# xmengli/H-DenseUNet

Measured on AMD Instinct MI355X. Metric: CT slices/sec fwd+bwd (2D 512^2), higher is better.
Workload: dtype bf16

## Files before the change

### h-denseunet_amd/csrc/conv_igemm.hip

```cpp
#include "conv_common.h"
#include "../../include/hdu.h"

template <typename T, int BM, int BN> struct BnbGeom {
  static constexpr int CH = Chunk<T>::CH;
  static constexpr int NCC = BN / CH;
  static constexpr int NCCP = NCC <= 4 ? 4 : (NCC <= 8 ? 8 : (NCC <= 16 ? 16 : 32));
  static constexpr int RSTEP = 256 / NCCP;
  static constexpr int IT = (BM + RSTEP - 1) / RSTEP;
  static constexpr bool EARLY = IT <= 8;
  static_assert(NCC <= 32, "tile shape");
};

template <bool SPLIT, typename T, int BM, int BN, int WAVES_M, int WAVES_N>
__device__ __forceinline__ void conv_igemm_body(const ConvK& p, char* smem) {
  constexpr int CH = Chunk<T>::CH;
  constexpr int BK = 8 * CH;
  constexpr int A_IT = BM / 32;
  constexpr int B_IT = (BN + 31) / 32;
  constexpr int WM = BM / WAVES_M;
  constexpr int WN = BN / WAVES_N;
  constexpr int TM = WM / 16;
  constexpr int TN = WN / 16;
  constexpr int STAGE = (BM + BN) * 128;
  static_assert(WAVES_M * WAVES_N == 4, "4 waves");
// ... 1571 lines not shown
          if constexpr (PRO) {
            const int cb = kt * BK + chunk * CH;
#pragma unroll
            for (int i = 0; i < TM; ++i) af[i] = pro_apply<T>(af[i], pro_ta + cb, pro_tb + cb, pro_lo);
          }
#pragma unroll
          for (int i = 0; i < TM; ++i)
#pragma unroll
            for (int j = 0; j < TN; ++j) acc[i][j] = Mma<T>::kgroup(bf[j], af[i], acc[i][j]);
        }
        if (!issue_first) issue(slot == 0 ? NS - 1 : slot - 1);
        slot = slot == NS - 1 ? 0 : slot + 1;
      }
      const int n0 = nt * BN;
      float* sdst = p.stats_partial ? p.stats_partial + (long long)((unsigned)mt % (unsigned)p.stats_slots) * 2 * p.Cout : nullptr;
#pragma unroll
      for (int j = 0; j < TN; ++j) {
        const int n = n0 + j * 16 + (lane >> 4) * 4;
        const bool n_ok = n < p.Cout;
        const int nc = n_ok ? n : 0;
        const f32x4 bias_v = has_bias ? *(const f32x4*)(p.bias + nc) : f32x4{0.f, 0.f, 0.f, 0.f};
        const f32x4 epa_v = has_epi ? *(const f32x4*)(p.epi_a + nc) : f32x4{1.f, 1.f, 1.f, 1.f};
        const f32x4 epb_v = has_epi ? *(const f32x4*)(p.epi_b + nc) : f32x4{0.f, 0.f, 0.f, 0.f};
        const f32x4 sh_v = sdst ? *(const f32x4*)(p.stats_shift + nc) : f32x4{0.f, 0.f, 0.f, 0.f};
        float s1[4] = {0.f, 0.f, 0.f, 0.f}, s2[4] = {0.f, 0.f, 0.f, 0.f};
#pragma unroll
        for (int i = 0; i < TM; ++i) {
          const long long m = (long long)mt * BM + wave * WM + i * 16 + (lane & 15);
          const bool ok = n_ok && m < p.M;
          T* dst = yp + (ok ? m * p.ldy + n : 0);
          float v[4] = {acc[i][j][0], acc[i][j][1], acc[i][j][2], acc[i][j][3]};
          if (has_bias) {
#pragma unroll
            for (int r = 0; r < 4; ++r) v[r] += bias_v[r];
          }
          if (drop) {
#pragma unroll
            for (int r = 0; r < 4; ++r) {
              const unsigned h = hdu_hash32((unsigned long long)m * (unsigned)p.Cout + (unsigned)(n + r), dseed);
              v[r] = h < p.drop_thresh ? v[r] * p.drop_scale : 0.f;
            }
          }
          if (has_epi) {
#pragma unroll
            for (int r = 0; r < 4; ++r) {
              v[r] = epa_v[r] * v[r] + epb_v[r];
              if (p.epi_relu) v[r] = v[r] > 0.f ? v[r] : 0.f;
            }
          }
          if (p.accumulate) {
            float old[4];
            Chunk<T>::load4(dst, old);
#pragma unroll
            for (int r = 0; r < 4; ++r) v[r] += old[r];
          }
          if (ok) Chunk<T>::store4(dst, v);
          if (sdst) {
#pragma unroll
            for (int r = 0; r < 4; ++r) {
              const float d = ok ? Chunk<T>::rounded(v[r]) - sh_v[r] : 0.f;
              s1[r] += d;
              s2[r] += d * d;
            }
          }
        }
        if (sdst) {
#pragma unroll
          for (int r = 0; r < 4; ++r) { s1[r] = hdu_row16_sum(s1[r]); s2[r] = hdu_row16_sum(s2[r]); }
          const int q = lane & 15;
          float mine = 0.f;
#pragma unroll
          for (int r = 0; r < 4; ++r) {
            mine = q == r ? s1[r] : mine;
            mine = q == 4 + r ? s2[r] : mine;
          }
          if (q < 8 && n_ok) atomicAdd(sdst + (q < 4 ? 0 : p.Cout) + n + (q & 3), mine);
        }
      }
    }
  }
  HDU_WAIT_VMCNT(0);
}

template <int KS, int BN, bool BNB = false, int NSA = 3>
__global__ __launch_bounds__(256) void conv_pw_bstat_kernel(ConvK p, int rows_per_wg) {
  typedef bf16_t T;
  constexpr int CH = 8, BM = 64;
  constexpr int PD = NSA - 1;
  constexpr int A_SLAB = BM * 128, A_STAGE = KS * A_SLAB;
  constexpr int B_SLAB = BN * 128, B_BYTES = KS * B_SLAB;
  constexpr int WM = 32, WN = BN / 2, TM = WM / 16, TN = WN / 16;
  constexpr int CROWB = WN * 2 + (BN == 64 && NSA == 2 ? 0 : 16), CST = WM * CROWB;
  static_assert(NSA == 2 || NSA == 3, "ring depth");
  constexpr int A_IT = BM / 32, B_IT = BN / 32, LA = KS * A_IT;
  static_assert(BN % 64 == 0 && KS >= 1 && KS <= 4, "shape");
  static_assert(B_BYTES + NSA * A_STAGE + 4 * CST <= 160 * 1024, "LDS");
  __shared__ __attribute__((aligned(16))) char smem[B_BYTES + NSA * A_STAGE + 4 * CST];
  char* Bsm = smem;
  char* Aring = smem + B_BYTES;

  const int tid = threadIdx.x;
  const int lane = tid & 63;
#ifdef HDU_EMU
  const int wave = tid >> 6;
#else
  const int wave = __builtin_amdgcn_readfirstlane(tid >> 6);
#endif
  const int wm = wave >> 1, wn = wave & 1;
  char* stg = smem + B_BYTES + NSA * A_STAGE + wave * CST;
  const int r0 = tid >> 3;
  const int kcl = (tid & 7) ^ (r0 & 7);
  unsigned brow = blockIdx.x, bcol = blockIdx.y;
  if (!(p.debug_flags & 2048)) {
    const unsigned lin = blockIdx.y * gridDim.x + blockIdx.x;
    const unsigned tix = xcd_tile_index(lin, gridDim.x * gridDim.y);
    bcol = tix % gridDim.y;
    brow = tix / gridDim.y;
  }
  const int n0 = (int)bcol * BN;
  const long long m_begin = (long long)brow * rows_per_wg;
  long long m_end = m_begin + rows_per_wg;
  if (m_end > p.M) m_end = p.M;
  const int ntiles = (int)((m_end - m_begin + BM - 1) / BM);
  if (ntiles <= 0) return;
  const hdu_bufsrd xsrd = hdu_make_srd(p.x, p.x_bytes);
  const hdu_bufsrd wsrd = hdu_make_srd(p.w, p.w_bytes);

#pragma unroll
  for (int ks = 0; ks < KS; ++ks)
#pragma unroll
    for (int j = 0; j < B_IT; ++j) {
      const int col = n0 + r0 + j * 32;
      const unsigned off = col < p.Cout ? (unsigned)(col * p.Ktot + ks * 64 + kcl * CH) * 2u : HDU_OOB;
      hdu_bufload_lds16(wsrd, off, Bsm + ks * B_SLAB + (j * 32 + wave * 8) * 128);
    }
  auto issue_tile = [&](int t) {
    char* As = Aring + (t % NSA) * A_STAGE;
#pragma unroll
    for (int i = 0; i < A_IT; ++i) {
      const long long m = m_begin + (long long)t * BM + r0 + i * 32;
#pragma unroll
      for (int ks = 0; ks < KS; ++ks) {
        const unsigned off = m < m_end ? (unsigned)((unsigned long long)m * (unsigned long long)p.ldx + ks * 64 + kcl * CH) * 2u : HDU_OOB;
        hdu_bufload_lds16(xsrd, off, As + ks * A_SLAB + (i * 32 + wave * 8) * 128);
      }
    }
  };
  T* __restrict__ yp = (T*)p.y;
  constexpr int NCCE = WN / CH;
  constexpr int EIT = WM * NCCE / 64;
  static_assert(EIT == 4 || EIT == 2, "the counted waits below name four / two registers per operand");
  const int ecc = lane % NCCE;
  const int en = n0 + wn * WN + ecc * CH;
  const bool en_ok = en < p.Cout;
  float ba[CH], bb[CH], bmu[CH], brs[CH], bs1[CH], bs2[CH];
  const bool bsums = BNB && p.bnb_partial != nullptr;
  if constexpr (BNB) {
    const int nc = en_ok ? en : 0;
    const float* pmu = bsums ? p.bnb_mean : p.bnb_a;
    const float* prs = bsums ? p.bnb_rstd : p.bnb_a;
#pragma unroll
    for (int j = 0; j < CH; j += 4) {
      const f32x4 va = *(const f32x4*)(p.bnb_a + nc + j), vb = *(const f32x4*)(p.bnb_b + nc + j);
      const f32x4 vm = *(const f32x4*)(pmu + nc + j), vr = *(const f32x4*)(prs + nc + j);
#pragma unroll
      for (int r = 0; r < 4; ++r) { ba[j + r] = va[r]; bb[j + r] = vb[r]; bmu[j + r] = bsums ? vm[r] : 0.f; brs[j + r] = bsums ? vr[r] : 0.f; }
    }
#pragma unroll
    for (int j = 0; j < CH; ++j) { bs1[j] = 0.f; bs2[j] = 0.f; }
  }
  const T* __restrict__ bup = (const T*)p.bnb_u;

  u32x4 uS[NSA][EIT], oS[NSA][EIT];
  u32x4 pst[EIT];
  unsigned poff[EIT];
#pragma unroll
  for (int it = 0; it < EIT; ++it) { poff[it] = HDU_OOB; pst[it] = u32x4{0u, 0u, 0u, 0u}; }
  const hdu_rawsrd ysrd = hdu_make_rawsrd(p.y, (unsigned)(((p.M - 1) * p.ldy + p.Cout) * 2));
  const hdu_rawsrd usrd = hdu_make_rawsrd(BNB ? p.bnb_u : p.y, (unsigned)(((p.M - 1) * (BNB ? p.bnb_ldu : p.ldy) + p.Cout) * 2));
  const unsigned ldu2 = (unsigned)p.bnb_ldu * 2u, ldy2 = (unsigned)p.ldy * 2u;
  const int erow = lane / NCCE;
  auto issue_chunks = [&](int t, u32x4 (&uv)[EIT], u32x4 (&ov)[EIT]) {
#pragma unroll
    for (int it = 0; it < EIT; ++it) {
      const long long m = m_begin + (long long)t * BM + wm * WM + erow + it * (64 / NCCE);
      const bool ok = en_ok && m < m_end;
      const unsigned uoff = ok ? (unsigned)m * ldu2 + (unsigned)en * 2u : HDU_OOB;
      const unsigned ooff = (ok && p.accumulate) ? (unsigned)m * ldy2 + (unsigned)en * 2u : HDU_OOB;
      HDU_ASYNC_BUFLOAD16(uv[it], usrd, uoff);
      HDU_ASYNC_BUFLOAD16(ov[it], ysrd, ooff);
    }
  };
  if constexpr (BNB) issue_chunks(0, uS[0], oS[0]);
  issue_tile(0);
  if constexpr (PD == 2) {
    if constexpr (BNB) issue_chunks(1, uS[1], oS[1]);
    issue_tile(1);
  }

  auto tile = [&](int t, u32x4 (&cuv)[EIT], u32x4 (&cov)[EIT], u32x4 (&nuv)[EIT], u32x4 (&nov)[EIT]) {
    if constexpr (BNB) hdu_wait_vmcnt_n<(PD - 1) * (LA + 2 * EIT)>(); else hdu_wait_vmcnt_n<(PD - 1) * LA>();
    HDU_RAW_BARRIER();
#pragma unroll
    for (int it = 0; it < EIT; ++it) hdu_bufstore16(ysrd, poff[it], pst[it]);
    if constexpr (BNB) issue_chunks(t + PD, nuv, nov);
    issue_tile(t + PD);
    f32x4 acc[TM][TN];
#pragma unroll
    for (int i = 0; i < TM; ++i)
#pragma unroll
      for (int j = 0; j < TN; ++j) acc[i][j] = f32x4{0.f, 0.f, 0.f, 0.f};
    const char* At = Aring + (t % NSA) * A_STAGE;
#pragma unroll
    for (int ks = 0; ks < KS; ++ks) {
      const char* As = At + ks * A_SLAB;
      const char* Bs = Bsm + ks * B_SLAB;
#pragma unroll
      for (int kg = 0; kg < 2; ++kg) {
        u32x4 af[TM], bf[TN];
        const int chunk = kg * 4 + (lane >> 4);
#pragma unroll
        for (int i = 0; i < TM; ++i) af[i] = *(const u32x4*)(As + lds_chunk_off(wm * WM + i * 16 + (lane & 15), chunk));
#pragma unroll
        for (int j = 0; j < TN; ++j) bf[j] = *(const u32x4*)(Bs + lds_chunk_off(wn * WN + j * 16 + (lane & 15), chunk));
#pragma unroll
        for (int i = 0; i < TM; ++i)
#pragma unroll
          for (int j = 0; j < TN; ++j) acc[i][j] = Mma<T>::kgroup(bf[j], af[i], acc[i][j]);
      }
    }
#pragma unroll
    for (int i = 0; i < TM; ++i)
#pragma unroll
      for (int j = 0; j < TN; ++j) {
        const float v[4] = {acc[i][j][0], acc[i][j][1], acc[i][j][2], acc[i][j][3]};
        Chunk<T>::store4((T*)(stg + (i * 16 + (lane & 15)) * CROWB) + j * 16 + (lane >> 4) * 4, v);
      }
    HDU_WAVE_LDS_SYNC();
    if constexpr (BNB) {
      constexpr int NUSE = LA + PD * (LA + 2 * EIT);
      if constexpr (EIT == 4) {
        hdu_wait_vmcnt_regs4<NUSE>(cuv[0], cuv[1], cuv[2], cuv[3]);
        hdu_wait_vmcnt_regs4<NUSE>(cov[0], cov[1], cov[2], cov[3]);
      } else {
        hdu_wait_vmcnt_regs4<NUSE>(cuv[0], cuv[1], cov[0], cov[1]);
      }
    }
#pragma unroll
    for (int it = 0; it < EIT; ++it) {
      const int q = lane + it * 64;
      const int row = q / NCCE, cc = q % NCCE;
      const long long m = m_begin + (long long)t * BM + wm * WM + row;
      const int n = n0 + wn * WN + cc * CH;
      const u32x4 v = *(const u32x4*)(stg + row * CROWB + cc * 16);
      const bool ok = m < m_end && n < p.Cout;
      poff[it] = ok ? (unsigned)m * ldy2 + (unsigned)n * 2u : HDU_OOB;
      if constexpr (BNB) {
        float dz[CH], u[CH], o[CH];
        Chunk<T>::unpack(v, dz);
        Chunk<T>::unpack(cuv[it], u);
#pragma unroll
        for (int j = 0; j < CH; ++j) {
          const float sj = ba[j] * u[j] + bb[j];
          const float g = (ok && (!p.bnb_relu || sj > 0.f)) ? dz[j] : 0.f;
          bs1[j] += g;
          bs2[j] += g * ((u[j] - bmu[j]) * brs[j]);
          o[j] = ba[j] * g;
        }
        if (p.accumulate) {
          float old[CH];
          Chunk<T>::unpack(cov[it], old);
#pragma unroll
          for (int j = 0; j < CH; ++j) o[j] += old[j];
        }
        pst[it] = Chunk<T>::pack(o);
      } else {
        pst[it] = v;
      }
    }
    HDU_WAVE_LDS_SYNC();
  };
  if constexpr (NSA == 3) {
    for (int t = 0; t < ntiles; t += 3) {
      tile(t, uS[0], oS[0], uS[2], oS[2]);
      if (t + 1 < ntiles) tile(t + 1, uS[1], oS[1], uS[0], oS[0]);
      if (t + 2 < ntiles) tile(t + 2, uS[2], oS[2], uS[1], oS[1]);
    }
  } else {
    for (int t = 0; t < ntiles; t += 2) {
      tile(t, uS[0], oS[0], uS[1], oS[1]);
      if (t + 1 < ntiles) tile(t + 1, uS[1], oS[1], uS[0], oS[0]);
    }
  }
#pragma unroll
  for (int it = 0; it < EIT; ++it) hdu_bufstore16(ysrd, poff[it], pst[it]);
  hdu_wait_vmcnt_n<0>();
  if constexpr (BNB) {
    if (bsums) {
#pragma unroll
      for (int mask = NCCE; mask < 64; mask <<= 1) {
#pragma unroll
        for (int j = 0; j < CH; ++j) { bs1[j] += __shfl_xor(bs1[j], mask); bs2[j] += __shfl_xor(bs2[j], mask); }
      }
      float* dst = p.bnb_partial + (long long)(brow % (unsigned)p.bnb_slots) * 2 * p.Cout;
      if (lane < NCCE && en_ok) {
#pragma unroll
        for (int j = 0; j < CH; ++j) {
          atomicAdd(dst + en + j, bs1[j]);
          atomicAdd(dst + p.Cout + en + j, bs2[j]);
        }
      }
    }
  }
}

template <int BCO, bool PW, int NCT = 1>
__device__ __forceinline__ void wgrad_dma_body(const ConvK& p, float* __restrict__ dw, long long rows_per_split,
                                               unsigned bid, char* smem) {
  typedef bf16_t T;
  constexpr int CH = 8;
  constexpr int PX = 64;
  constexpr int BKC = 128;
  constexpr int XROWB = 256;
  constexpr int DROWB = 128;
  constexpr int TM = BCO / 16;
  constexpr int TN = 2;
  constexpr int STAGE = PX * (XROWB + NCT * DROWB);

  const int tid = threadIdx.x;
  const int lane = tid & 63;
#ifdef HDU_EMU
  const int wave = tid >> 6;
#else
  const int wave = __builtin_amdgcn_readfirstlane(tid >> 6);
#endif
  const T* __restrict__ xp = (const T*)p.x;
  const T* __restrict__ dyp = (const T*)p.y;
  const char* zero = (const char*)hdu_zero_page;
  const bool ups = (p.ud | p.uh | p.uw) != 0;

  unsigned wbx, wby, wbz;
  if (!(p.debug_flags & 256)) bid = xcd_tile_index(bid, (unsigned)(p.wg_gx * p.wg_gy * p.wg_gz));
  if (!wgrad_block(p, bid, &wbx, &wby, &wbz)) return;
  const int kcol0 = (int)wbx * BKC;
  const int co0 = (int)wby * BCO * NCT;
  const long long m_begin = (long long)wbz * rows_per_split;
  long long m_end = m_begin + rows_per_split;
  if (m_end > p.M) m_end = p.M;

  const int pxl = tid >> 4;
  const int fx = (pxl & 3) | ((pxl >> 1) & 4);
  const int xp16 = tid & 15;
  const int kcc = ((((xp16 >> 1) ^ fx) << 1) | (xp16 & 1));
  const int kk = kcol0 + kcc * CH;
  const bool kvalid = kk < p.Ktot;
  int c = 0, kd = 0, kh = 0, kw = 0;
  if (kvalid) {
    const int tap = kk / p.Cin;
    c = kk - tap * p.Cin;
    kw = tap % p.KW;
    const int t = tap / p.KW;
    kh = t % p.KH;
    kd = t / p.KH;
  }
  int sn[4], sod[4], soh[4], sow[4];
#pragma unroll
  for (int i = 0; i < 4; ++i) {
    if (PW) { sn[i] = sod[i] = soh[i] = sow[i] = 0; continue; }
    const long long m = m_begin + pxl + i * 16;
    const unsigned mu = (unsigned)m;
    const int ow = (int)(mu % (unsigned)p.Wo);
    unsigned t = mu / (unsigned)p.Wo;
    const int oh = (int)(t % (unsigned)p.Ho);
    t /= (unsigned)p.Ho;
    sod[i] = (int)(t % (unsigned)p.Do);
    sn[i] = (int)(t / (unsigned)p.Do);
    soh[i] = oh;
    sow[i] = ow;
  }
  const int dpx0 = tid >> 3;
  const int gd = ((dpx0 >> 1) & 1) | (((dpx0 >> 3) & 1) << 1);
  const int dp16 = tid & 7;
  const int dcl = ((((dp16 >> 1) ^ gd) << 1) | (dp16 & 1));
  bool dvalid[NCT];
#pragma unroll
  for (int t = 0; t < NCT; ++t) dvalid[t] = dcl * CH < BCO && co0 + t * BCO + dcl * CH < p.Cout;

  auto issue_tile = [&](int buf, long long mt) {
    char* Xt = smem + buf * STAGE;
    char* Dt = Xt + PX * XROWB;
#pragma unroll
    for (int i = 0; i < 4; ++i) {
      const long long m = mt + pxl + i * 16;
      const char* g;
      if (PW) {
        g = (kvalid && m < m_end) ? (const char*)(xp + m * p.ldx + c) : zero;
// ... 1048 lines not shown
  return items >= min_items && k.M < (1ll << 31) - 256;
}

template <typename T, int BN>
static void launch_pers(const ConvK& k, hipStream_t s) {
  const int tiles_m = (int)((k.M + 255) / 256), tiles_n = (k.Cout + BN - 1) / BN;
  const int cus = g_tuning[HDU_TUNE_PERS] > 1 ? g_tuning[HDU_TUNE_PERS] : 256;
  long long items = (long long)tiles_m * tiles_n;
  const dim3 grid((unsigned)(items < cus ? items : cus));
  if (k.pro_a != nullptr) {
    const int cap = pers_table_cap(BN, k.Cin);
    if (cap == HDU_PRO_CSMALL) {
      if constexpr (3 * (256 + BN) * 128 + 8 * HDU_PRO_CSMALL <= 160 * 1024)
        HDU_LAUNCH((conv_igemm_pers_kernel<T, BN, HDU_PRO_CSMALL>), grid, dim3(512), 0, s, k, tiles_m, tiles_n);
    } else {
      if constexpr (3 * (256 + BN) * 128 + 8 * HDU_PRO_CMAX <= 160 * 1024)
        HDU_LAUNCH((conv_igemm_pers_kernel<T, BN, HDU_PRO_CMAX>), grid, dim3(512), 0, s, k, tiles_m, tiles_n);
    }
  } else {
    HDU_LAUNCH((conv_igemm_pers_kernel<T, BN, 0>), grid, dim3(512), 0, s, k, tiles_m, tiles_n);
  }
}

template <typename T>
static void dispatch_igemm(const ConvK& k, size_t skb, hipStream_t s) {
  int bm, bn;
  choose_igemm(k, &bm, &bn);
  if (bm == 128 && igemm_pers_ok(k, bn)) {
    switch (bn) {
      case 128: launch_pers<T, 128>(k, s); return;
      case 96: launch_pers<T, 96>(k, s); return;
      case 64: launch_pers<T, 64>(k, s); return;
      case 48: launch_pers<T, 48>(k, s); return;
      default: launch_pers<T, 32>(k, s); return;
    }
  }
  if (bm == 64) dispatch_igemm_bn<T, 64>(k, bn, skb, s);
  else dispatch_igemm_bn<T, 128>(k, bn, skb, s);
}

bool hdu_halo_wide_taken(const ConvK& k, int dtype);
const char* hdu_halo_wide_name(const ConvK& k, int dtype);
bool hdu_halo_wide_launch(const ConvK& k, int dtype, hipStream_t s);
bool hdu_stem_wgrad_taken(const ConvK& k, int dtype);
bool hdu_stem_wgrad_launch(const ConvK& k, int dtype, float* dw, hipStream_t s);

static bool fprop_halo_ok(const ConvK& k, int dtype) {
  return dtype == HDU_BF16 && k.bnb_u == nullptr && !g_tuning[HDU_TUNE_NO_HALO_FPROP] && k.pro_a == nullptr && k.skip == nullptr && k.KD == 1 &&
         k.KH == 3 && k.KW == 3 && k.sd == 1 && k.sh == 1 && k.sw == 1 && k.pd == 0 && k.ph == 1 && k.pw == 1 &&
         (k.ud | k.uh | k.uw) == 0 && k.Di == 1 && k.Cin % 8 == 0 && k.We >= 32 && k.He >= 4 &&
         k.Do == 1 && k.Ho == k.He && k.Wo == k.We &&
         k.Cin >= 128 && k.Cout <= 96 &&
         (long long)k.N * ((k.He + 3) / 4) * ((k.We + 31) / 32) * k.M_layer / k.M >= (g_tuning[HDU_TUNE_HALO_MIN_TILES] > 0 ? g_tuning[HDU_TUNE_HALO_MIN_TILES] : 128);
}

static int choose_halo_bn(const ConvK& k) {
  const int cands[4] = {96, 64, 48, 32};
  int best = 64;
  long long best_cost = -1;
  for (int i = 0; i < 4; ++i) {
    const int c = cands[i];
    const long long cost = (long long)((k.Cout + c - 1) / c) * (c + 24);
    if (best_cost < 0 || cost < best_cost) { best_cost = cost; best = c; }
  }
  return best;
}

template <int BN>
static void launch_halo_fprop(const ConvK& k, hipStream_t s) {
  const unsigned tiles = (unsigned)(k.N * ((k.He + 3) / 4) * ((k.We + 31) / 32));
  HDU_LAUNCH((conv_halo_fprop_kernel<BN>), dim3(tiles, (unsigned)((k.Cout + BN - 1) / BN)), dim3(256), 0, s, k);
}

static bool pw_bstat_ok(const ConvK& k, int dtype) {
  return dtype == HDU_BF16 && !g_tuning[HDU_TUNE_NO_PW_BSTAT] && k.KD * k.KH * k.KW == 1 && k.sd == 1 && k.sh == 1 && k.sw == 1 &&
         (k.pd | k.ph | k.pw) == 0 && (k.ud | k.uh | k.uw) == 0 && k.pro_a == nullptr && k.skip == nullptr && k.bias == nullptr &&
         k.epi_a == nullptr && k.stats_partial == nullptr && (k.bnb_u != nullptr ? (!g_tuning[HDU_TUNE_NO_PW_BSTAT_BNB] && !(k.bnb_relu & 6)) : !k.accumulate) &&
         k.drop_scale == 0.f &&
         (k.Ktot == 128 || k.Ktot == 192) && k.Cout >= 256 && k.M >= 64 && k.x_bytes != 0 &&
         (k.M - 1) * k.ldy + k.Cout < (1ll << 31) && (k.bnb_u == nullptr || (k.M - 1) * k.bnb_ldu + k.Cout < (1ll << 31)) &&
         (long long)k.Cout * k.Ktot * 2 < (1ll << 31) && k.Do == k.De && k.Ho == k.He && k.Wo == k.We;
}

template <int BN, int NSA>
static void launch_pw_bstat_form(const ConvK& k, int target, hipStream_t s) {
  const unsigned ny = (unsigned)((k.Cout + BN - 1) / BN);
  long long splits = target / (long long)ny;
  if (splits < 1) splits = 1;
  const long long tiles = (k.M + 63) / 64;
  if (splits > tiles) splits = tiles;
  const long long rows = ((tiles + splits - 1) / splits) * 64;
  const unsigned gx = (unsigned)((k.M + rows - 1) / rows);
  if (k.bnb_u != nullptr) {
    if (k.Ktot == 192) HDU_LAUNCH((conv_pw_bstat_kernel<3, BN, true, NSA>), dim3(gx, ny), dim3(256), 0, s, k, (int)rows);
    else HDU_LAUNCH((conv_pw_bstat_kernel<2, BN, true, NSA>), dim3(gx, ny), dim3(256), 0, s, k, (int)rows);
    return;
  }
  if (k.Ktot == 192) HDU_LAUNCH((conv_pw_bstat_kernel<3, BN, false, NSA>), dim3(gx, ny), dim3(256), 0, s, k, (int)rows);
  else HDU_LAUNCH((conv_pw_bstat_kernel<2, BN, false, NSA>), dim3(gx, ny), dim3(256), 0, s, k, (int)rows);
}

static int pw_bstat_form(const ConvK& k) {
  const int f = g_tuning[HDU_TUNE_PW_BSTAT_FORM];
  if (f == 1 || f == 2) return f;
  return k.bnb_u != nullptr ? 2 : 1;
}

static void launch_pw_bstat(const ConvK& k, hipStream_t s) {
  const int wgs = g_tuning[HDU_TUNE_PW_BSTAT_WGS];
  if (pw_bstat_form(k) == 2) launch_pw_bstat_form<64, 2>(k, wgs > 0 ? wgs : 512, s);
  else launch_pw_bstat_form<128, 3>(k, wgs > 0 ? wgs : 256, s);
}

extern "C" int hdu_conv_fprop(const hdu_conv_desc* d, void* stream) {
  ConvK k;
  if (int e = fill_convk(d, &k, false)) return e;
  if (!d->y) return hdu_set_error(HDU_ERR_ARG, "conv_fprop: null output");
  if (k.M == 0) return 0;
  if (k.y_ds && !hdu_halo_wide_taken(k, d->dtype))
    return hdu_set_error(HDU_ERR_ARG, "conv_fprop: y_ds needs a launch that a halo-wide configuration takes");
  if (pw_bstat_ok(k, d->dtype)) {
    launch_pw_bstat(k, (hipStream_t)stream);
    return hdu_check_launch("conv_fprop(pointwise, filter-stationary)");
  }
  if (hdu_halo_wide_launch(k, d->dtype, (hipStream_t)stream)) return hdu_check_launch("conv_fprop(halo, wide)");
  if (fprop_halo_ok(k, d->dtype)) {
    switch (choose_halo_bn(k)) {
      case 96: launch_halo_fprop<96>(k, (hipStream_t)stream); break;
      case 64: launch_halo_fprop<64>(k, (hipStream_t)stream); break;
      case 48: launch_halo_fprop<48>(k, (hipStream_t)stream); break;
      default: launch_halo_fprop<32>(k, (hipStream_t)stream); break;
    }
    return hdu_check_launch("conv_fprop(halo)");
  }
  if (d->dtype == HDU_BF16) dispatch_igemm<bf16_t>(k, d->splitk_ws_bytes, (hipStream_t)stream);
  else dispatch_igemm<float>(k, d->splitk_ws_bytes, (hipStream_t)stream);
  return hdu_check_launch("conv_fprop");
}

extern "C" size_t hdu_conv_splitk_ws_bytes(const hdu_conv_desc* d) {
  ConvK k;
  if (fill_convk(d, &k, false)) return 0;
  if (k.M == 0 || pw_bstat_ok(k, d->dtype) || hdu_halo_wide_taken(k, d->dtype) || fprop_halo_ok(k, d->dtype) || (k.pro_a != nullptr && !igemm_pro_dma_ok(k)) || k.skip != nullptr) return 0;
  int bm, bn;
  choose_igemm(k, &bm, &bn);
  if (bm == 128 && igemm_pers_ok(k, bn)) return 0;
  const long long nblk = ((k.M + bm - 1) / bm) * ((k.Cout + bn - 1) / bn);
  const long long nblk_layer = ((k.M_layer + bm - 1) / bm) * ((k.Cout + bn - 1) / bn);
  const int stage = (bm + ((bn + 31) / 32) * 32) * 128;
  const int nsd = stage * 6 <= 160 * 1024 ? 6 : 4;
  if (!igemm_ring_ok(nblk_layer, k.Ktot, stage, nsd)) return 0;
  const int bk = d->dtype == HDU_BF16 ? 64 : 32;
  size_t need;
  choose_splitk(nblk_layer, (k.Ktot + bk - 1) / bk, bm, bn, ring_wgs_per_cu(bm, d->dtype == HDU_BF16), &need);
  return need / (size_t)nblk_layer * (size_t)nblk;
}

template <typename T, int BCO>
static void launch_wgrad(const ConvK& k, float* dw, hipStream_t s) {
  constexpr int PX = 8 * Chunk<T>::CH;
  const unsigned gx = (unsigned)((k.Ktot + 127) / 128), gy = (unsigned)((k.Cout + BCO - 1) / BCO);
  const long long target = g_tuning[HDU_TUNE_WGRAD_TARGET_WGS] > 0 ? g_tuning[HDU_TUNE_WGRAD_TARGET_WGS] : 1024;
  long long want = target / ((long long)gx * gy);
  if (want < 1) want = 1;
  long long steps = (k.M + PX - 1) / PX;
  if (want > steps) want = steps;
  long long steps_per = (steps + want - 1) / want;
  const long long rows_per = steps_per * PX;
  const unsigned gz = (unsigned)((k.M + rows_per - 1) / rows_per);
  HDU_LAUNCH((conv_wgrad_kernel<T, BCO>), dim3(gx, gy, gz), dim3(256), 0, s, k, dw, rows_per);
}

static int choose_wgrad(const ConvK& k) {
  const int cands[3] = {64, 48, 32};
  int best = 64;
  long long best_cost = -1;
  for (int i = 0; i < 3; ++i) {
    const long long padded = (long long)((k.Cout + cands[i] - 1) / cands[i]) * cands[i];
    if (best_cost < 0 || padded < best_cost) { best_cost = padded; best = cands[i]; }
  }
  return best;
}

static unsigned wgrad_grid(const ConvK& k) { return (unsigned)k.wg_gz * (unsigned)(k.wg_gx * k.wg_gy); }


static bool wgrad_pointwise(const ConvK& k) {
  return k.KD * k.KH * k.KW == 1 && k.sd == 1 && k.sh == 1 && k.sw == 1 && (k.pd | k.ph | k.pw) == 0 &&
         (k.ud | k.uh | k.uw) == 0;
}

static int wgrad_nct(const ConvK& k, int BCO) {
  if (g_tuning[HDU_TUNE_WGRAD_NCT] == 1 || !wgrad_pointwise(k) || BCO != 64) return 1;
// ... 208 lines not shown
    for (int a = 0; a < 3; ++a) {
      g.step[a] = S[a];
      int kmax = K[a] - 1;
      if (S[a] == 2 && ((kmax - r[a] - P[a]) & 1)) --kmax;
      g.kmax[a] = kmax;
      g.nt[a] = kmax < 0 ? 0 : kmax / S[a] + 1;
      if (g.nt[a] <= 0) return -1;
    }
    g.dst_off = off;
    off += (long long)Cin * g.nt[0] * g.nt[1] * g.nt[2] * Cout;
  }
  return 0;
}

extern "C" int hdu_stride2_dgrad_filters(int dtype, const float* w_master, int Cout, int KD, int KH, int KW, int Cin, int sd,
                                         int sh, int sw, int pd, int ph, int pw, void* w_out, void* stream) {
  ParityTable tab;
  if (!w_master || !w_out || Cout <= 0 || Cin <= 0 || parity_table(KD, KH, KW, sd, sh, sw, pd, ph, pw, Cin, Cout, &tab))
    return hdu_set_error(HDU_ERR_ARG, "stride2_dgrad_filters: bad args (strides must be 1 or 2)");
  const dim3 grid(64, (unsigned)tab.n);
  if (dtype == HDU_BF16)
    HDU_LAUNCH((stride2_filter_kernel<bf16_t>), grid, dim3(256), 0, (hipStream_t)stream, w_master, Cout, KD, KH, KW, Cin, tab, (bf16_t*)w_out);
  else if (dtype == HDU_F32)
    HDU_LAUNCH((stride2_filter_kernel<float>), grid, dim3(256), 0, (hipStream_t)stream, w_master, Cout, KD, KH, KW, Cin, tab, (float*)w_out);
  else
    return hdu_set_error(HDU_ERR_ARG, "stride2_dgrad_filters: bad dtype");
  return hdu_check_launch("stride2_dgrad_filters");
}

extern "C" int hdu_parity_interleave(int dtype, const void* cls, int N, int Di, int Hi, int Wi, int C, int sd, int sh, int sw,
                                     void* dx, int64_t lddx, int accumulate, void* stream) {
  const int ch = dtype == HDU_BF16 ? 8 : 4;
  if (!cls || !dx || N <= 0 || C <= 0 || C % ch || lddx % ch || Di % sd || Hi % sh || Wi % sw || (sd != 1 && sd != 2) ||
      (sh != 1 && sh != 2) || (sw != 1 && sw != 2))
    return hdu_set_error(HDU_ERR_ARG, "parity_interleave: bad args (dims must be multiples of the strides)");
  const long long total = (long long)N * Di * Hi * Wi * (C / ch);
  long long blocks = (total + 255) / 256;
  if (blocks > 8192) blocks = 8192;
  if (dtype == HDU_BF16)
    HDU_LAUNCH((parity_interleave_kernel<bf16_t>), dim3((unsigned)blocks), dim3(256), 0, (hipStream_t)stream, (const bf16_t*)cls,
               N, Di, Hi, Wi, C, sd, sh, sw, (bf16_t*)dx, (long long)lddx, accumulate);
  else if (dtype == HDU_F32)
    HDU_LAUNCH((parity_interleave_kernel<float>), dim3((unsigned)blocks), dim3(256), 0, (hipStream_t)stream, (const float*)cls, N,
               Di, Hi, Wi, C, sd, sh, sw, (float*)dx, (long long)lddx, accumulate);
  else
    return hdu_set_error(HDU_ERR_ARG, "parity_interleave: bad dtype");
  return hdu_check_launch("parity_interleave");
}

extern "C" int hdu_weight_prep(int dtype, const float* w_master, int Cout, int T, int Cin, void* w_f, void* w_d,
                               void* stream) {
  if (!w_master || Cout <= 0 || T <= 0 || Cin <= 0) return hdu_set_error(HDU_ERR_ARG, "weight_prep: bad args");
  const long long total = (long long)Cout * T * Cin;
  long long blocks = (total + 255) / 256;
  if (blocks > 2048) blocks = 2048;
  if (dtype == HDU_BF16)
    HDU_LAUNCH((weight_prep_kernel<bf16_t>), dim3((unsigned)blocks), dim3(256), 0, (hipStream_t)stream, w_master,
               Cout, T, Cin, (bf16_t*)w_f, (bf16_t*)w_d);
  else if (dtype == HDU_F32)
    HDU_LAUNCH((weight_prep_kernel<float>), dim3((unsigned)blocks), dim3(256), 0, (hipStream_t)stream, w_master,
               Cout, T, Cin, (float*)w_f, (float*)w_d);
  else
    return hdu_set_error(HDU_ERR_ARG, "weight_prep: bad dtype");
  return hdu_check_launch("weight_prep");
}

#include <cstdio>
extern "C" int hdu_conv_kernel_name(const hdu_conv_desc* d, int op, char* buf, size_t buflen) {
  ConvK k;
  if (int e = fill_convk(d, &k, op == 1)) return e;
  if (!buf || buflen < 8) return hdu_set_error(HDU_ERR_ARG, "conv_kernel_name: bad buffer");
  const char* t = d->dtype == HDU_BF16 ? "unsigned short" : "float";
  if (op == 1) {
    const bool dma = wgrad_dma_ok(k);
    const bool pw = k.KD * k.KH * k.KW == 1 && k.sd == 1 && k.sh == 1 && k.sw == 1 && (k.pd | k.ph | k.pw) == 0 &&
                    (k.ud | k.uh | k.uw) == 0;
    if (hdu_stem_wgrad_taken(k, d->dtype)) snprintf(buf, buflen, "conv_stem_wgrad_kernel");
    else if (d->dtype == HDU_BF16 && wgrad_halo_ok(k)) snprintf(buf, buflen, "conv_wgrad_halo_kernel<%d>", choose_wgrad(k));
    else if (d->dtype == HDU_BF16 && dma) snprintf(buf, buflen, "conv_wgrad_dma_kernel<%d, %s>", choose_wgrad(k), pw ? "true" : "false");
    else if (d->dtype == HDU_BF16) snprintf(buf, buflen, "conv_wgrad_tr_kernel<%d>", choose_wgrad(k));
    else snprintf(buf, buflen, "conv_wgrad_kernel<float, %d>", choose_wgrad(k));
  } else if (pw_bstat_ok(k, d->dtype)) {
    if (pw_bstat_form(k) == 2) snprintf(buf, buflen, "conv_pw_bstat_kernel<%d, 64, %s, 2>", k.Ktot / 64, k.bnb_u ? "true" : "false");
    else snprintf(buf, buflen, "conv_pw_bstat_kernel<%d, 128, %s, 3>", k.Ktot / 64, k.bnb_u ? "true" : "false");
  } else if (hdu_halo_wide_taken(k, d->dtype)) {
    snprintf(buf, buflen, "%s", hdu_halo_wide_name(k, d->dtype));
  } else if (fprop_halo_ok(k, d->dtype)) {
    snprintf(buf, buflen, "conv_halo_fprop_kernel<%d>", choose_halo_bn(k));
  } else {
    int bm, bn;
    choose_igemm(k, &bm, &bn);
    if (bm == 128 && igemm_pers_ok(k, bn)) {
      snprintf(buf, buflen, "conv_igemm_pers_kernel<%s, %d, %d>", t, bn, k.pro_a ? pers_table_cap(bn, k.Cin) : 0);
      return 0;
    }
    const int wm = (bn >= 128) ? 2 : ((bm == 64 && (bn == 64 || bn == 32)) ? 2 : 4);
    const bool prodma = igemm_pro_dma_ok(k);
    const bool dma = prodma || (k.pro_a == nullptr && k.skip == nullptr && k.vec_out);
    const long long nblk = ((k.M_layer + bm - 1) / bm) * ((k.Cout + bn - 1) / bn);
    const int mode = g_tuning[HDU_TUNE_DMA_STAGES];
    const int stage = (bm + ((bn + 31) / 32) * 32) * 128;
    const int nsd = stage * 6 <= 160 * 1024 ? 6 : 4;
    const bool ring = dma && igemm_ring_ok(nblk, k.Ktot, stage, nsd);
    int nsr = (nsd == 6 && ring_wgs_per_cu(bm, d->dtype == HDU_BF16) == 2) ? 3 : nsd;
    const int proc = prodma ? (k.Cin <= HDU_PRO_CSMALL ? HDU_PRO_CSMALL : HDU_PRO_CMAX) : 0;
    if (prodma && nsr * stage + 8 * proc > 160 * 1024) nsr = nsr == 6 ? 4 : 3;
    const char* fast = igemm_fast_ok(k) ? "true" : "false";
    const char* bnb = k.bnb_u != nullptr ? "true" : "false";
    if (ring) snprintf(buf, buflen, "conv_igemm_ring_kernel<%s, %d, %d, %d, %d, %d, %s, %s, %d>", t, bm, bn, wm, 4 / wm, nsr, fast, bnb, proc);
    else if (dma) snprintf(buf, buflen, "conv_igemm_dma_kernel<%s, %d, %d, %d, %d, %s, %s, %d>", t, bm, bn, wm, 4 / wm, fast, bnb, proc);
    else snprintf(buf, buflen, "conv_igemm_kernel<%s, %d, %d, %d, %d>", t, bm, bn, wm, 4 / wm);
  }
  return 0;
}

extern "C" int hdu_weight_prep_batched(int dtype, const hdu_prep_entry* table, int n, int64_t total_tiles,
                                       const float* master_base, void* wc_base, void* stream) {
  if (!table || n <= 0 || total_tiles <= 0 || !master_base || !wc_base)
    return hdu_set_error(HDU_ERR_ARG, "weight_prep_batched: bad args");
  if (dtype == HDU_BF16)
    HDU_LAUNCH((weight_prep_batched_kernel<bf16_t>), dim3((unsigned)((total_tiles + HDU_PREP_TPW - 1) / HDU_PREP_TPW)), dim3(256), 0,
               (hipStream_t)stream, table, n, master_base, (bf16_t*)wc_base, (long long)total_tiles);
  else if (dtype == HDU_F32)
    HDU_LAUNCH((weight_prep_batched_kernel<float>), dim3((unsigned)((total_tiles + HDU_PREP_TPW - 1) / HDU_PREP_TPW)), dim3(256), 0,
               (hipStream_t)stream, table, n, master_base, (float*)wc_base, (long long)total_tiles);
  else
    return hdu_set_error(HDU_ERR_ARG, "weight_prep_batched: bad dtype");
  return hdu_check_launch("weight_prep_batched");
}
```

Before: 548.0.

## Add 8-wave pointwise bstat conv variant with swizzled staging for large layers

Factors the pointwise filter-stationary conv kernel into a body templated on wave count and adds a 512-thread, 8-wave variant with BN=128 that splits N across four waves. When each wave's N slice is 32 wide, the output staging buffer uses an XOR swizzle instead of padding. The new variant is chosen by default for large-M BN-backward cases and for wide Cout forward cases. It trades more waves per workgroup and more latency hiding against a larger LDS footprint and possibly lower occupancy.

```diff
diff --git a/h-denseunet_amd/csrc/conv_igemm.hip b/h-denseunet_amd/csrc/conv_igemm.hip
--- a/h-denseunet_amd/csrc/conv_igemm.hip
+++ b/h-denseunet_amd/csrc/conv_igemm.hip
@@ -1677,20 +1677,33 @@
   HDU_WAIT_VMCNT(0);
 }
 
-template <int KS, int BN, bool BNB = false, int NSA = 3>
-__global__ __launch_bounds__(256) void conv_pw_bstat_kernel(ConvK p, int rows_per_wg) {
+template <int KS, int BN, bool BNB, int NSA, int NW>
+struct PwBstatCfg {
+  static constexpr int BM = 64, WM = 32, WN = BN / (NW / 2);
+  static constexpr int A_STAGE = KS * BM * 128, B_BYTES = KS * BN * 128;
+  static constexpr bool SWZ = WN == 32;
+  static constexpr int CROWB = WN * 2 + (SWZ ? 0 : 16), CST = WM * CROWB;
+  static constexpr int SMEM = B_BYTES + NSA * A_STAGE + NW * CST;
+  static_assert(SMEM <= 160 * 1024, "LDS");
+};
+
+template <int KS, int BN, bool BNB, int NSA, int NW>
+__device__ __forceinline__ void pw_bstat_body(const ConvK& p, int rows_per_wg, char* smem) {
   typedef bf16_t T;
-  constexpr int CH = 8, BM = 64;
+  typedef PwBstatCfg<KS, BN, BNB, NSA, NW> Cfg;
+  constexpr int CH = 8, BM = Cfg::BM;
   constexpr int PD = NSA - 1;
   constexpr int A_SLAB = BM * 128, A_STAGE = KS * A_SLAB;
   constexpr int B_SLAB = BN * 128, B_BYTES = KS * B_SLAB;
-  constexpr int WM = 32, WN = BN / 2, TM = WM / 16, TN = WN / 16;
-  constexpr int CROWB = WN * 2 + (BN == 64 && NSA == 2 ? 0 : 16), CST = WM * CROWB;
+  constexpr int NWN = NW / 2;
+  constexpr int WM = Cfg::WM, WN = Cfg::WN, TM = WM / 16, TN = WN / 16;
+  constexpr int CROWB = Cfg::CROWB, CST = Cfg::CST;
+  constexpr bool SWZ = Cfg::SWZ;
   static_assert(NSA == 2 || NSA == 3, "ring depth");
-  constexpr int A_IT = BM / 32, B_IT = BN / 32, LA = KS * A_IT;
-  static_assert(BN % 64 == 0 && KS >= 1 && KS <= 4, "shape");
-  static_assert(B_BYTES + NSA * A_STAGE + 4 * CST <= 160 * 1024, "LDS");
-  __shared__ __attribute__((aligned(16))) char smem[B_BYTES + NSA * A_STAGE + 4 * CST];
+  static_assert(NW == 4 || NW == 8, "waves");
+  constexpr int RIT = NW * 8;
+  constexpr int A_IT = BM / RIT, B_IT = BN / RIT, LA = KS * A_IT;
+  static_assert(BN % 64 == 0 && BM % RIT == 0 && BN % RIT == 0 && KS >= 1 && KS <= 4, "shape");
   char* Bsm = smem;
   char* Aring = smem + B_BYTES;
 
@@ -1701,7 +1714,7 @@
 #else
   const int wave = __builtin_amdgcn_readfirstlane(tid >> 6);
 #endif
-  const int wm = wave >> 1, wn = wave & 1;
+  const int wm = wave / NWN, wn = wave % NWN;
   char* stg = smem + B_BYTES + NSA * A_STAGE + wave * CST;
   const int r0 = tid >> 3;
   const int kcl = (tid & 7) ^ (r0 & 7);
@@ -1725,19 +1738,19 @@
   for (int ks = 0; ks < KS; ++ks)
 #pragma unroll
     for (int j = 0; j < B_IT; ++j) {
-      const int col = n0 + r0 + j * 32;
+      const int col = n0 + r0 + j * RIT;
       const unsigned off = col < p.Cout ? (unsigned)(col * p.Ktot + ks * 64 + kcl * CH) * 2u : HDU_OOB;
-      hdu_bufload_lds16(wsrd, off, Bsm + ks * B_SLAB + (j * 32 + wave * 8) * 128);
+      hdu_bufload_lds16(wsrd, off, Bsm + ks * B_SLAB + (j * RIT + wave * 8) * 128);
     }
   auto issue_tile = [&](int t) {
     char* As = Aring + (t % NSA) * A_STAGE;
 #pragma unroll
     for (int i = 0; i < A_IT; ++i) {
-      const long long m = m_begin + (long long)t * BM + r0 + i * 32;
+      const long long m = m_begin + (long long)t * BM + r0 + i * RIT;
 #pragma unroll
       for (int ks = 0; ks < KS; ++ks) {
         const unsigned off = m < m_end ? (unsigned)((unsigned long long)m * (unsigned long long)p.ldx + ks * 64 + kcl * CH) * 2u : HDU_OOB;
-        hdu_bufload_lds16(xsrd, off, As + ks * A_SLAB + (i * 32 + wave * 8) * 128);
+        hdu_bufload_lds16(xsrd, off, As + ks * A_SLAB + (i * RIT + wave * 8) * 128);
       }
     }
   };
@@ -1829,7 +1842,11 @@
 #pragma unroll
       for (int j = 0; j < TN; ++j) {
         const float v[4] = {acc[i][j][0], acc[i][j][1], acc[i][j][2], acc[i][j][3]};
-        Chunk<T>::store4((T*)(stg + (i * 16 + (lane & 15)) * CROWB) + j * 16 + (lane >> 4) * 4, v);
+        const int prow = i * 16 + (lane & 15);
+        const int pc = j * 2 + (lane >> 5);
+        char* dst = SWZ ? stg + prow * CROWB + ((pc ^ ((prow >> 1) & 3)) * 16 + ((lane >> 4) & 1) * 8)
+                        : stg + prow * CROWB + (j * 16 + (lane >> 4) * 4) * 2;
+        Chunk<T>::store4((T*)dst, v);
       }
     HDU_WAVE_LDS_SYNC();
     if constexpr (BNB) {
@@ -1847,7 +1864,7 @@
       const int row = q / NCCE, cc = q % NCCE;
       const long long m = m_begin + (long long)t * BM + wm * WM + row;
       const int n = n0 + wn * WN + cc * CH;
-      const u32x4 v = *(const u32x4*)(stg + row * CROWB + cc * 16);
+      const u32x4 v = *(const u32x4*)(stg + row * CROWB + (SWZ ? cc ^ ((row >> 1) & 3) : cc) * 16);
       const bool ok = m < m_end && n < p.Cout;
       poff[it] = ok ? (unsigned)m * ldy2 + (unsigned)n * 2u : HDU_OOB;
       if constexpr (BNB) {
@@ -1907,6 +1924,18 @@
       }
     }
   }
+}
+
+template <int KS, int BN, bool BNB = false, int NSA = 3>
+__global__ __launch_bounds__(256) void conv_pw_bstat_kernel(ConvK p, int rows_per_wg) {
+  __shared__ __attribute__((aligned(16))) char smem[PwBstatCfg<KS, BN, BNB, NSA, 4>::SMEM];
+  pw_bstat_body<KS, BN, BNB, NSA, 4>(p, rows_per_wg, smem);
+}
+
+template <int KS, bool BNB>
+__global__ __launch_bounds__(512) void conv_pw_bstat_kernel_w8(ConvK p, int rows_per_wg) {
+  __shared__ __attribute__((aligned(16))) char smem[PwBstatCfg<KS, 128, BNB, 3, 8>::SMEM];
+  pw_bstat_body<KS, 128, BNB, 3, 8>(p, rows_per_wg, smem);
 }
 
 template <int BCO, bool PW, int NCT = 1>
@@ -3121,7 +3150,7 @@
          (long long)k.Cout * k.Ktot * 2 < (1ll << 31) && k.Do == k.De && k.Ho == k.He && k.Wo == k.We;
 }
 
-template <int BN, int NSA>
+template <int BN, int NSA, int NW = 4>
 static void launch_pw_bstat_form(const ConvK& k, int target, hipStream_t s) {
   const unsigned ny = (unsigned)((k.Cout + BN - 1) / BN);
   long long splits = target / (long long)ny;
@@ -3130,6 +3159,16 @@
   if (splits > tiles) splits = tiles;
   const long long rows = ((tiles + splits - 1) / splits) * 64;
   const unsigned gx = (unsigned)((k.M + rows - 1) / rows);
+  if constexpr (NW == 8) {
+    if (k.bnb_u != nullptr) {
+      if (k.Ktot == 192) HDU_LAUNCH((conv_pw_bstat_kernel_w8<3, true>), dim3(gx, ny), dim3(512), 0, s, k, (int)rows);
+      else HDU_LAUNCH((conv_pw_bstat_kernel_w8<2, true>), dim3(gx, ny), dim3(512), 0, s, k, (int)rows);
+    } else {
+      if (k.Ktot == 192) HDU_LAUNCH((conv_pw_bstat_kernel_w8<3, false>), dim3(gx, ny), dim3(512), 0, s, k, (int)rows);
+      else HDU_LAUNCH((conv_pw_bstat_kernel_w8<2, false>), dim3(gx, ny), dim3(512), 0, s, k, (int)rows);
+    }
+    return;
+  }
   if (k.bnb_u != nullptr) {
     if (k.Ktot == 192) HDU_LAUNCH((conv_pw_bstat_kernel<3, BN, true, NSA>), dim3(gx, ny), dim3(256), 0, s, k, (int)rows);
     else HDU_LAUNCH((conv_pw_bstat_kernel<2, BN, true, NSA>), dim3(gx, ny), dim3(256), 0, s, k, (int)rows);
@@ -3141,13 +3180,16 @@
 
 static int pw_bstat_form(const ConvK& k) {
   const int f = g_tuning[HDU_TUNE_PW_BSTAT_FORM];
-  if (f == 1 || f == 2) return f;
-  return k.bnb_u != nullptr ? 2 : 1;
+  if (f >= 1 && f <= 3) return f;
+  if (k.bnb_u != nullptr) return k.M >= 131072 ? 3 : 2;
+  return k.Cout >= 720 ? 3 : 1;
 }
 
 static void launch_pw_bstat(const ConvK& k, hipStream_t s) {
   const int wgs = g_tuning[HDU_TUNE_PW_BSTAT_WGS];
-  if (pw_bstat_form(k) == 2) launch_pw_bstat_form<64, 2>(k, wgs > 0 ? wgs : 512, s);
+  const int form = pw_bstat_form(k);
+  if (form == 2) launch_pw_bstat_form<64, 2>(k, wgs > 0 ? wgs : 512, s);
+  else if (form == 3) launch_pw_bstat_form<128, 3, 8>(k, wgs > 0 ? wgs : 256, s);
   else launch_pw_bstat_form<128, 3>(k, wgs > 0 ? wgs : 256, s);
 }
 
@@ -3522,6 +3564,7 @@
     else snprintf(buf, buflen, "conv_wgrad_kernel<float, %d>", choose_wgrad(k));
   } else if (pw_bstat_ok(k, d->dtype)) {
     if (pw_bstat_form(k) == 2) snprintf(buf, buflen, "conv_pw_bstat_kernel<%d, 64, %s, 2>", k.Ktot / 64, k.bnb_u ? "true" : "false");
+    else if (pw_bstat_form(k) == 3) snprintf(buf, buflen, "conv_pw_bstat_kernel_w8<%d, %s>", k.Ktot / 64, k.bnb_u ? "true" : "false");
     else snprintf(buf, buflen, "conv_pw_bstat_kernel<%d, 128, %s, 3>", k.Ktot / 64, k.bnb_u ? "true" : "false");
   } else if (hdu_halo_wide_taken(k, d->dtype)) {
     snprintf(buf, buflen, "%s", hdu_halo_wide_name(k, d->dtype));
```

After: 548.2, median of 3. About the same (+0.0%).
